# iwa-shi/CRDR

Measured on AMD Instinct MI355X. Metric: stage-3 training img/s at 256x256, higher is better.
Workload: dtype fp32; 1 GPU; config/crdr_stage_3.yaml -b 16: full GAN step (G + 5x CLIC21GVAE D + LPIPS-Alex, random-init weights), rate index cycled 0..4; global_batch=16, crop=256, parallelism=dp1

## Files before the change

crdr_amd/csrc/igemm.hip:

```cpp
#include <algorithm>
#include <type_traits>

#include "algo_id.hpp"
#include "igemm_kernel.hpp"
#include "wino.hpp"

namespace crdr {

extern template __global__ void igemm_kernel<4, 1, 1, 1, false, 0, false>(const IgemmArgs, const IgemmTaps, const IgemmGroup);
extern template __global__ void igemm_kernel<4, 1, 1, 2, false, 0, false>(const IgemmArgs, const IgemmTaps, const IgemmGroup);
extern template __global__ void igemm_kernel<4, 1, 1, 3, false, 0, false>(const IgemmArgs, const IgemmTaps, const IgemmGroup);
extern template __global__ void igemm_kernel<4, 1, 1, 4, false, 0, false>(const IgemmArgs, const IgemmTaps, const IgemmGroup);
extern template __global__ void igemm_kernel<4, 1, 1, 5, false, 0, false>(const IgemmArgs, const IgemmTaps, const IgemmGroup);
extern template __global__ void igemm_kernel<4, 1, 1, 6, false, 0, false>(const IgemmArgs, const IgemmTaps, const IgemmGroup);
extern template __global__ void igemm_kernel<4, 1, 1, 7, false, 0, false>(const IgemmArgs, const IgemmTaps, const IgemmGroup);
extern template __global__ void igemm_kernel<4, 1, 2, 2, false, 0, false>(const IgemmArgs, const IgemmTaps, const IgemmGroup);
extern template __global__ void igemm_kernel<4, 1, 2, 3, false, 0, false>(const IgemmArgs, const IgemmTaps, const IgemmGroup);
extern template __global__ void igemm_kernel<4, 1, 2, 4, false, 0, false>(const IgemmArgs, const IgemmTaps, const IgemmGroup);
extern template __global__ void igemm_kernel<2, 2, 2, 2, false, 0, false>(const IgemmArgs, const IgemmTaps, const IgemmGroup);
extern template __global__ void igemm_kernel<2, 2, 1, 1, false, 0, false>(const IgemmArgs, const IgemmTaps, const IgemmGroup);
extern template __global__ void igemm_kernel<2, 2, 1, 2, false, 0, false>(const IgemmArgs, const IgemmTaps, const IgemmGroup);
extern template __global__ void igemm_kernel<2, 2, 1, 3, false, 0, false>(const IgemmArgs, const IgemmTaps, const IgemmGroup);
extern template __global__ void igemm_kernel<2, 2, 1, 4, false, 0, false>(const IgemmArgs, const IgemmTaps, const IgemmGroup);
extern template __global__ void igemm_kernel<1, 4, 1, 1, false, 0, false>(const IgemmArgs, const IgemmTaps, const IgemmGroup);
extern template __global__ void igemm_kernel<1, 4, 1, 2, false, 0, false>(const IgemmArgs, const IgemmTaps, const IgemmGroup);
extern template __global__ void igemm_kernel<4, 2, 1, 1, false, 0, false>(const IgemmArgs, const IgemmTaps, const IgemmGroup);
extern template __global__ void igemm_kernel<4, 2, 1, 2, false, 0, false>(const IgemmArgs, const IgemmTaps, const IgemmGroup);
extern template __global__ void igemm_kernel<4, 2, 1, 3, false, 0, false>(const IgemmArgs, const IgemmTaps, const IgemmGroup);
extern template __global__ void igemm_kernel<4, 2, 2, 1, false, 0, false>(const IgemmArgs, const IgemmTaps, const IgemmGroup);
extern template __global__ void igemm_kernel<4, 2, 2, 2, false, 0, false>(const IgemmArgs, const IgemmTaps, const IgemmGroup);
extern template __global__ void igemm_kernel<2, 4, 1, 1, false, 0, false>(const IgemmArgs, const IgemmTaps, const IgemmGroup);
extern template __global__ void igemm_kernel<2, 4, 2, 1, false, 0, false>(const IgemmArgs, const IgemmTaps, const IgemmGroup);
extern template __global__ void igemm_kernel<2, 4, 1, 2, false, 0, false>(const IgemmArgs, const IgemmTaps, const IgemmGroup);
extern template __global__ void igemm_kernel<2, 2, 2, 1, false, 0, false>(const IgemmArgs, const IgemmTaps, const IgemmGroup);
extern template __global__ void igemm_kernel<2, 2, 2, 3, false, 0, false>(const IgemmArgs, const IgemmTaps, const IgemmGroup);
extern template __global__ void igemm_kernel<4, 1, 1, 1, true, 0, false>(const IgemmArgs, const IgemmTaps, const IgemmGroup);
extern template __global__ void igemm_kernel<4, 1, 1, 2, true, 0, false>(const IgemmArgs, const IgemmTaps, const IgemmGroup);
extern template __global__ void igemm_kernel<4, 1, 2, 2, true, 0, false>(const IgemmArgs, const IgemmTaps, const IgemmGroup);
extern template __global__ void igemm_kernel<2, 2, 2, 2, true, 0, false>(const IgemmArgs, const IgemmTaps, const IgemmGroup);
extern template __global__ void igemm_kernel<4, 2, 1, 1, true, 0, false>(const IgemmArgs, const IgemmTaps, const IgemmGroup);
extern template __global__ void igemm_kernel<4, 2, 1, 2, true, 0, false>(const IgemmArgs, const IgemmTaps, const IgemmGroup);
extern template __global__ void igemm_kernel<4, 2, 2, 1, true, 0, false>(const IgemmArgs, const IgemmTaps, const IgemmGroup);
extern template __global__ void igemm_kernel<4, 2, 2, 2, true, 0, false>(const IgemmArgs, const IgemmTaps, const IgemmGroup);
extern template __global__ void igemm_kernel<2, 4, 2, 1, true, 0, false>(const IgemmArgs, const IgemmTaps, const IgemmGroup);
extern template __global__ void igemm_kernel<4, 1, 1, 1, false, 3, false>(const IgemmArgs, const IgemmTaps, const IgemmGroup);
extern template __global__ void igemm_kernel<4, 1, 1, 2, false, 3, false>(const IgemmArgs, const IgemmTaps, const IgemmGroup);
extern template __global__ void igemm_kernel<4, 1, 1, 3, false, 3, false>(const IgemmArgs, const IgemmTaps, const IgemmGroup);
extern template __global__ void igemm_kernel<4, 1, 1, 4, false, 3, false>(const IgemmArgs, const IgemmTaps, const IgemmGroup);
extern template __global__ void igemm_kernel<4, 1, 1, 5, false, 3, false>(const IgemmArgs, const IgemmTaps, const IgemmGroup);
extern template __global__ void igemm_kernel<4, 1, 1, 6, false, 3, false>(const IgemmArgs, const IgemmTaps, const IgemmGroup);
extern template __global__ void igemm_kernel<4, 1, 1, 7, false, 3, false>(const IgemmArgs, const IgemmTaps, const IgemmGroup);
extern template __global__ void igemm_kernel<4, 1, 2, 2, false, 3, false>(const IgemmArgs, const IgemmTaps, const IgemmGroup);
extern template __global__ void igemm_kernel<4, 1, 2, 3, false, 3, false>(const IgemmArgs, const IgemmTaps, const IgemmGroup);
extern template __global__ void igemm_kernel<4, 1, 2, 4, false, 3, false>(const IgemmArgs, const IgemmTaps, const IgemmGroup);
extern template __global__ void igemm_kernel<2, 2, 2, 2, false, 3, false>(const IgemmArgs, const IgemmTaps, const IgemmGroup);
extern template __global__ void igemm_kernel<2, 2, 1, 1, false, 3, false>(const IgemmArgs, const IgemmTaps, const IgemmGroup);
extern template __global__ void igemm_kernel<2, 2, 1, 2, false, 3, false>(const IgemmArgs, const IgemmTaps, const IgemmGroup);
extern template __global__ void igemm_kernel<2, 2, 1, 3, false, 3, false>(const IgemmArgs, const IgemmTaps, const IgemmGroup);
extern template __global__ void igemm_kernel<2, 2, 1, 4, false, 3, false>(const IgemmArgs, const IgemmTaps, const IgemmGroup);
extern template __global__ void igemm_kernel<1, 4, 1, 1, false, 3, false>(const IgemmArgs, const IgemmTaps, const IgemmGroup);
extern template __global__ void igemm_kernel<1, 4, 1, 2, false, 3, false>(const IgemmArgs, const IgemmTaps, const IgemmGroup);
extern template __global__ void igemm_kernel<4, 2, 1, 1, false, 3, false>(const IgemmArgs, const IgemmTaps, const IgemmGroup);
extern template __global__ void igemm_kernel<4, 2, 1, 2, false, 3, false>(const IgemmArgs, const IgemmTaps, const IgemmGroup);
extern template __global__ void igemm_kernel<4, 2, 1, 3, false, 3, false>(const IgemmArgs, const IgemmTaps, const IgemmGroup);
extern template __global__ void igemm_kernel<4, 2, 2, 1, false, 3, false>(const IgemmArgs, const IgemmTaps, const IgemmGroup);
extern template __global__ void igemm_kernel<4, 2, 2, 2, false, 3, false>(const IgemmArgs, const IgemmTaps, const IgemmGroup);
extern template __global__ void igemm_kernel<2, 4, 1, 1, false, 3, false>(const IgemmArgs, const IgemmTaps, const IgemmGroup);
extern template __global__ void igemm_kernel<2, 4, 2, 1, false, 3, false>(const IgemmArgs, const IgemmTaps, const IgemmGroup);
extern template __global__ void igemm_kernel<2, 4, 1, 2, false, 3, false>(const IgemmArgs, const IgemmTaps, const IgemmGroup);
extern template __global__ void igemm_kernel<2, 2, 2, 1, false, 3, false>(const IgemmArgs, const IgemmTaps, const IgemmGroup);
extern template __global__ void igemm_kernel<2, 2, 2, 3, false, 3, false>(const IgemmArgs, const IgemmTaps, const IgemmGroup);
extern template __global__ void igemm_kernel<4, 1, 1, 2, false, 6, false>(const IgemmArgs, const IgemmTaps, const IgemmGroup);
extern template __global__ void igemm_kernel<4, 1, 1, 4, false, 6, false>(const IgemmArgs, const IgemmTaps, const IgemmGroup);
extern template __global__ void igemm_kernel<2, 2, 2, 2, false, 6, false>(const IgemmArgs, const IgemmTaps, const IgemmGroup);
extern template __global__ void igemm_kernel<2, 2, 1, 1, false, 6, false>(const IgemmArgs, const IgemmTaps, const IgemmGroup);
extern template __global__ void igemm_kernel<2, 2, 1, 2, false, 6, false>(const IgemmArgs, const IgemmTaps, const IgemmGroup);
extern template __global__ void igemm_kernel<2, 2, 1, 3, false, 6, false>(const IgemmArgs, const IgemmTaps, const IgemmGroup);
extern template __global__ void igemm_kernel<4, 2, 1, 2, false, 6, false>(const IgemmArgs, const IgemmTaps, const IgemmGroup);
extern template __global__ void igemm_kernel<2, 4, 2, 1, false, 6, false>(const IgemmArgs, const IgemmTaps, const IgemmGroup);
extern template __global__ void igemm_kernel<2, 2, 2, 1, false, 6, false>(const IgemmArgs, const IgemmTaps, const IgemmGroup);
extern template __global__ void igemm_kernel<4, 1, 1, 1, false, 0, true>(const IgemmArgs, const IgemmTaps, const IgemmGroup);
extern template __global__ void igemm_kernel<4, 1, 1, 2, false, 0, true>(const IgemmArgs, const IgemmTaps, const IgemmGroup);
extern template __global__ void igemm_kernel<4, 1, 1, 3, false, 0, true>(const IgemmArgs, const IgemmTaps, const IgemmGroup);
extern template __global__ void igemm_kernel<4, 1, 1, 4, false, 0, true>(const IgemmArgs, const IgemmTaps, const IgemmGroup);
extern template __global__ void igemm_kernel<4, 1, 1, 5, false, 0, true>(const IgemmArgs, const IgemmTaps, const IgemmGroup);
extern template __global__ void igemm_kernel<4, 1, 1, 6, false, 0, true>(const IgemmArgs, const IgemmTaps, const IgemmGroup);
extern template __global__ void igemm_kernel<4, 1, 1, 7, false, 0, true>(const IgemmArgs, const IgemmTaps, const IgemmGroup);
// ... 372 lines not shown
    CRDR_REQUIRE(al16(q.x) && al16(q.w), "conv2d: x and w must be 16-byte aligned (problem %d)", g);
    CRDR_REQUIRE(!(flags & CRDR_EPI_BIAS) || q.bias, "conv2d: BIAS flag without bias (problem %d)", g);
    CRDR_REQUIRE(!(flags & CRDR_EPI_PREADD) || q.pre, "conv2d: PREADD flag without pre (problem %d)", g);
    CRDR_REQUIRE(!(flags & (CRDR_EPI_RELUMASK | CRDR_EPI_LRELUMASK)) || q.mask, "conv2d: mask flag without mask (problem %d)", g);
    CRDR_REQUIRE(!(flags & CRDR_EPI_RES) || q.res, "conv2d: RES flag without res (problem %d)", g);
    CRDR_REQUIRE(!(flags & CRDR_EPI_COLSUM) || q.cs, "conv2d: COLSUM flag without cs (problem %d)", g);
  }
  return 0;
}

static bool rows_aligned(const crdr_conv_desc* d, const crdr_conv_io* ios, int G) {
  const bool res = d->flags & CRDR_EPI_RES, gate = d->flags & CRDR_EPI_GATE, pre = d->flags & CRDR_EPI_PREADD;
  const bool mask = d->flags & (CRDR_EPI_RELUMASK | CRDR_EPI_LRELUMASK);
  bool v = d->ldy % 4 == 0 && (!res || d->ldres % 4 == 0) && (!pre || d->ldpre % 4 == 0) && (!mask || d->ldmask % 4 == 0) &&
           (!gate || (d->ldg % 4 == 0 && al16(ios[0].gx) && al16(ios[0].gt) && al16(ios[0].sig)));
  for (int g = 0; g < G; ++g) {
    const crdr_conv_io& q = ios[g];
    v = v && al16(q.y) && (!res || al16(q.res)) && (!pre || al16(q.pre)) && (!mask || al16(q.mask));
  }
  return v;
}

static bool fast_epilogue_ok(const IgemmArgs& a, bool vec_epi) {
  const long long span_px = (256 / std::max(a.GW, 1) + 2) * (long long)std::max(a.so, 1) * a.OW + a.OW;
  const long long span = span_px * std::max(std::max(a.ldy, a.ldres), a.ldmask) * 4;
  return vec_epi && a.Cout % 4 == 0 && span < (1ll << 31) && !(a.flags & (CRDR_EPI_GATE | CRDR_EPI_PREADD | CRDR_EPI_ACCUM));
}

static void bind_io(Plan* pl, const crdr_conv_io* ios, int G, void* ws, IgemmGroup* grp) {
  IgemmArgs& a = pl->a;
  const crdr_conv_io& io = ios[0];
  a.x = io.x; a.w = io.w; a.y = io.y;
  a.counters = (int*)ws;
  a.ws = (float*)ws + CRDR_CONV_TICKETS;
  a.bias = io.bias; a.vec2 = io.vec2; a.res = io.res; a.scale = io.scale; a.shift = io.shift;
  a.gx = io.gx; a.gt = io.gt; a.sig = io.sig; a.pre = io.pre; a.mask = io.mask; a.cs = io.cs;
  memset(grp, 0, sizeof(*grp));
  for (int g = 0; g < G; ++g) {
    const crdr_conv_io& q = ios[g];
    grp->x[g] = q.x; grp->w[g] = q.w; grp->y[g] = q.y; grp->bias[g] = q.bias; grp->pre[g] = q.pre; grp->mask[g] = q.mask;
    grp->res[g] = q.res; grp->cs[g] = q.cs;
  }
}

static int launch_conv(const crdr_conv_desc* d, const crdr_conv_io* ios, int G, void* ws, size_t ws_bytes, crdr_stream_t s,
                       float* ucache = nullptr, size_t ucache_bytes = 0, int ucache_valid = 0) {
  Plan pl;
  if (int rc = build_plan(d, &pl, G)) return rc;
  if (pl.a.M == 0) return 0;
  if (int rc = check_io(d, ios, G, pl.ws_bytes, ws_bytes)) return rc;
  const bool vec_epi = rows_aligned(d, ios, G);
  if (pl.stream >= 0 && !vec_epi && d->reserved == 0) {
    if (int rc = build_plan(d, &pl, G, true)) return rc;
  }
  IgemmGroup grp;
  bind_io(&pl, ios, G, ws, &grp);
  IgemmArgs& a = pl.a;
  a.vec_epi = vec_epi ? 1 : 0;
  a.fast_epi = fast_epilogue_ok(a, vec_epi) ? 1 : 0;
  if (pl.wino != WinoKernel::None) {
    const bool f4 = pl.wino == WinoKernel::F4;
    void* prof = profile_begin(as_stream(s));
    if (f4) {
      const size_t u_bytes = wino4_workspace(d, G, 1);
      float* u = (float*)ws + CRDR_CONV_TICKETS;
      if (ucache) {
        CRDR_REQUIRE(ucache_bytes >= u_bytes, "conv2d: filter cache of %zu bytes, the launch needs %zu", ucache_bytes, u_bytes);
        u = ucache;
      }
      float* slabs = (float*)ws + CRDR_CONV_TICKETS + u_bytes / 4;
      if (int rc = wino4_launch(d, a, pl.t, grp, G, u, slabs, a.nsplit, ucache && ucache_valid, as_stream(s))) return rc;
    } else if (int rc = wino_launch(d, pl.wino == WinoKernel::F2Pairs, a, pl.t, grp, G, (float*)ws + CRDR_CONV_TICKETS, as_stream(s))) return rc;
    profile_end(f4 ? (d->kh == 5 ? 6 : 5) : 3, G * crdr_conv2d_flops(d), prof, as_stream(s));
    return 0;
  }
  if (pl.stream >= 0) {
    CRDR_REQUIRE(a.vec_epi, "conv2d: the streaming kernel needs 16-byte aligned operand rows");
    void* prof = profile_begin(as_stream(s));
    stream_launch(pl.stream, a, pl.sa, grp, pl.grid.x, pl.lds, as_stream(s));
    CRDR_CHECK_LAUNCH("gemm1x1_kernel");
    profile_end(0, G * crdr_conv2d_flops(d), prof, as_stream(s));
    return 0;
  }
  const TileCfg& t = kCfgs[pl.cfg];
  const TileForm form = a.smallc ? kTapMajor : ((d->flags & CRDR_CONV_BF16X3) ? kBf3 : ((d->flags & CRDR_CONV_BF16X6) ? kBf6 : ((a.fast_epi && a.nsplit == 1) ? kFast : kPlain)));
  const IgemmKern kern = t.kern[form];
  CRDR_REQUIRE(kern, "conv2d: config %d has no kernel for this precision", pl.cfg);
  static std::atomic<bool> attr_done[kNumTileForms][64];
  allow_full_lds(attr_done[form][pl.cfg], kern);
  void* prof = profile_begin(as_stream(s));
  hipLaunchKernelGGL(kern, pl.grid, dim3(64 * t.wm * t.wn), pl.lds, as_stream(s), a, pl.t, grp);
  CRDR_CHECK_LAUNCH("igemm_kernel");
  profile_end(0, G * crdr_conv2d_flops(d), prof, as_stream(s));
  return 0;
}

extern "C" int crdr_conv2d(const crdr_conv_desc* d, const crdr_conv_io* io, void* ws, size_t ws_bytes,
                           crdr_stream_t s) {
  CRDR_REQUIRE(d && io, "conv2d: null descriptor");
  return launch_conv(d, io, 1, ws, ws_bytes, s);
}

extern "C" int crdr_conv2d_grouped(const crdr_conv_desc* d, const crdr_conv_io* ios, int G, void* ws, size_t ws_bytes,
                                   crdr_stream_t s) {
  CRDR_REQUIRE(d && ios, "conv2d_grouped: null descriptor");
  CRDR_REQUIRE(G >= 1 && G <= CRDR_MAX_GROUP, "conv2d_grouped: %d problems (1..%d)", G, CRDR_MAX_GROUP);
  return launch_conv(d, ios, G, ws, ws_bytes, s);
}

extern "C" size_t crdr_conv2d_filter_cache_bytes(const crdr_conv_desc* d, int G) {
  Plan pl;
  if (!d || G < 1 || G > CRDR_MAX_GROUP || build_plan(d, &pl, G) || pl.wino != WinoKernel::F4) return 0;
  return wino4_workspace(d, G, 1);
}

extern "C" int crdr_conv2d_filter_item(const crdr_conv_desc* d, int G, crdr_w4_filter_item* item) {
  CRDR_REQUIRE(d && item, "conv2d_filter_item: null pointer");
  CRDR_REQUIRE(G >= 1 && G <= CRDR_MAX_GROUP, "conv2d_filter_item: %d problems (1..%d)", G, CRDR_MAX_GROUP);
  Plan pl;
  if (int rc = build_plan(d, &pl, G)) return rc;
  CRDR_REQUIRE(pl.wino == WinoKernel::F4, "conv2d_filter_item: the descriptor's `reserved` does not force the F(4x4, 3x3) kernel");
  return wino4_filter_item(d, pl.t, G, item);
}

extern "C" int crdr_w4_filters_batched(const crdr_w4_filter_item* items, const int64_t* prefix, const int64_t* meta, crdr_stream_t s) {
  CRDR_REQUIRE(items && prefix && meta, "w4_filters_batched: null pointer");
  return wino4_filters_batched(items, reinterpret_cast<const long long*>(prefix), reinterpret_cast<const long long*>(meta), as_stream(s));
}

extern "C" int crdr_conv2d_grouped_ex(const crdr_conv_desc* d, const crdr_conv_io* ios, int G, void* ws, size_t ws_bytes, float* filter_cache,
                                      size_t filter_cache_bytes, int filter_cache_valid, crdr_stream_t s) {
  CRDR_REQUIRE(d && ios, "conv2d_grouped_ex: null descriptor");
  CRDR_REQUIRE(G >= 1 && G <= CRDR_MAX_GROUP, "conv2d_grouped_ex: %d problems (1..%d)", G, CRDR_MAX_GROUP);
  CRDR_REQUIRE(!filter_cache || (reinterpret_cast<uintptr_t>(filter_cache) & 15) == 0, "conv2d_grouped_ex: the filter cache must be 16-byte aligned");
  return launch_conv(d, ios, G, ws, ws_bytes, s, filter_cache, filter_cache_bytes, filter_cache_valid);
}
```

crdr_amd/hip/lib.py:

```python
from __future__ import annotations

import ctypes as C
import os
import subprocess
import threading

_HERE = os.path.dirname(os.path.abspath(__file__))
CSRC_DIR = os.path.normpath(os.path.join(_HERE, "..", "csrc"))
LIB_PATH = os.environ.get("CRDR_HIP_LIB") or os.path.normpath(os.path.join(_HERE, "..", "_lib", "libcrdr_hip.so"))

c_float_p = C.POINTER(C.c_float)
c_void_p = C.c_void_p


class ConvDesc(C.Structure):
    _fields_ = [(n, C.c_int32) for n in (
        "N", "H", "W", "C", "OH", "OW", "OC", "kh", "kw", "stride", "pad", "transposed", "ldx", "ldy",
        "wrows", "wcols", "flags", "ldres", "ldg", "wlayout", "reserved", "ldpre", "ldmask")]


class ConvIO(C.Structure):
    _fields_ = [(n, c_void_p) for n in (
        "x", "w", "y", "bias", "vec2", "res", "scale", "shift", "gx", "gt", "sig", "pre", "mask", "cs")]

# ... 12 lines not shown
class EbwdDesc(C.Structure):
    _fields_ = [("M", C.c_int64)] + [(n, C.c_int32) for n in (
        "C", "flags", "lddout", "ldout", "lddz", "ldgres", "ldg")]


class WgradJob(C.Structure):
    _fields_ = [("slab", c_void_p), ("g", c_void_p)] + [(n, C.c_int32) for n in (
        "PC", "QC", "gI", "gJ", "T", "nsplit", "smallj", "accumulate", "gJtot", "reserved")]


class LinearGroup(C.Structure):
    _fields_ = [(n, c_void_p * 16) for n in ("w", "b", "y", "dy", "dw", "db")] + [("O", C.c_int32 * 16)]


class PackItem(C.Structure):
    _fields_ = [("src", c_void_p), ("dst", c_void_p)] + [(n, C.c_int32) for n in (
        "I", "J", "T", "rows", "cols", "mode", "srcJ", "dld")] + [("tstride", C.c_int64)]


class W4FilterItem(C.Structure):
    _fields_ = [("w", c_void_p * 16), ("u", c_void_p)] + [(n, C.c_int32) for n in (
        "G", "Cin", "Cout", "wrows", "wcols", "kchunks", "ntile", "nvar")] + [("widx", (C.c_int32 * 9) * 4), ("units", C.c_int64)]


class GdnDesc(C.Structure):
    _fields_ = [("M", C.c_int64)] + [(n, C.c_int32) for n in ("C", "ldx", "ldy", "inverse")] + [
        ("beta_min", C.c_float), ("reparam_offset", C.c_float)]


class ChannelNormDesc(C.Structure):
    _fields_ = [("M", C.c_int64)] + [(n, C.c_int32) for n in ("C", "ldx", "ldy", "ldres", "act")] + [
        ("slope", C.c_float), ("eps", C.c_float)]


class InstanceNormDesc(C.Structure):
    _fields_ = [("HW", C.c_int64)] + [(n, C.c_int32) for n in ("N", "C", "ldx", "ldy", "act")] + [("slope", C.c_float), ("eps", C.c_float)]


class GanLossDesc(C.Structure):
    _fields_ = [("n", C.c_int64), ("nq", C.c_int64), ("kind", C.c_int32), ("center", C.c_int32), ("target", C.c_float), ("sgn", C.c_float)]


class Upsample16Desc(C.Structure):
    _fields_ = [(n, C.c_int32) for n in ("N", "h", "w", "Cc", "ldi", "ldc", "ldo", "mode")]


class GcDesc2(C.Structure):
    _fields_ = [(n, C.c_int32) for n in ("N", "HW", "C", "ldy", "ldmu", "ldsigma", "ldyhat", "ldyhat2", "ldnoise", "ldlik",
                                         "ldgrad", "lddyhat", "Ctot", "c0")] + [
        ("scale_bound", C.c_float), ("likelihood_bound", C.c_float)]


class GcIO(C.Structure):
    _fields_ = [(n, c_void_p) for n in ("y", "mu", "sigma", "noise", "philox", "yhat", "yhat2", "lik_noisy", "lik_quant",
                                        "bits_noisy", "bits_quant", "gbits", "dyhat", "dy", "dmu", "dsigma", "ws")] + [
        ("ws_bytes", C.c_size_t)]


class EbwdIO(C.Structure):
    _fields_ = [(n, c_void_p) for n in (
        "dout", "out", "vec2", "scale", "shift", "gt", "sig", "dz", "gres", "dgt", "colsums", "dbias_accum")]


class GcDesc(C.Structure):
    _fields_ = [(n, C.c_int32) for n in ("N", "HW", "C", "ldy", "ldmu", "ldsigma", "ldyhat")] + [
        ("scale_bound", C.c_float), ("likelihood_bound", C.c_float)]


EPI_BIAS, EPI_RELU, EPI_LRELU, EPI_VEC2, EPI_RES, EPI_GATE, EPI_AFFINE, EPI_ACCUM = 1, 2, 4, 8, 16, 32, 64, 128
EPI_PREADD, EPI_RELUMASK, EPI_LRELUMASK, EPI_MASKOFF, EPI_COLSUM = 256, 512, 1024, 2048, 4096
CONV_NOSPLIT, CONV_BF16X3, WGRAD_BF16X3 = 8192, 16384, 1 << 16
CONV_BF16X6, WGRAD_BF16X6 = 32768, 1 << 17
WGRAD_SQUARE_Q = 1 << 18
MAX_GROUP = 16
EB_PARAMS = 58

_I, _I64, _F, _D, _P, _SZ = C.c_int, C.c_int64, C.c_float, C.c_double, c_void_p, C.c_size_t
SIGNATURES = {
    "crdr_last_error": (C.c_char_p, []),
    "crdr_version": (_I, []),
    "crdr_arch": (C.c_char_p, []),
    "crdr_profile_enable": (None, [_I]),
    "crdr_profile_read": (_I, [_I, C.POINTER(C.c_double), C.POINTER(C.c_double), C.POINTER(C.c_longlong)]),
    "crdr_conv2d_num_configs": (_I, []),
    "crdr_conv2d_num_stream_configs": (_I, []),
    "crdr_conv2d_num_wino_configs": (_I, []),
    "crdr_conv2d_wgrad_num_configs": (_I, []),
    "crdr_conv2d_wgrad_num_wino_configs": (_I, []),
    "crdr_conv2d_workspace": (_SZ, [C.POINTER(ConvDesc)]),
    "crdr_conv2d_choose_algo": (_I, [C.POINTER(ConvDesc), _I]),
    "crdr_conv2d": (_I, [C.POINTER(ConvDesc), C.POINTER(ConvIO), _P, _SZ, _P]),
    "crdr_conv2d_flops": (_D, [C.POINTER(ConvDesc)]),
    "crdr_conv2d_colsum_layout": (_I, [C.POINTER(ConvDesc), _I, C.POINTER(C.c_int), C.POINTER(C.c_int)]),
    "crdr_colsum_slab_rows": (_I, []),
    "crdr_colsum_finish_batched": (_I, [_P, _P, _P, _P, _P, _P]),
    "crdr_conv2d_grouped_workspace": (_SZ, [C.POINTER(ConvDesc), _I]),
    "crdr_conv2d_grouped": (_I, [C.POINTER(ConvDesc), _P, _I, _P, _SZ, _P]),
    "crdr_conv2d_filter_cache_bytes": (_SZ, [C.POINTER(ConvDesc), _I]),
    "crdr_conv2d_grouped_ex": (_I, [C.POINTER(ConvDesc), _P, _I, _P, _SZ, _P, _SZ, _I, _P]),
    "crdr_conv2d_filter_item": (_I, [C.POINTER(ConvDesc), _I, C.POINTER(W4FilterItem)]),
    "crdr_w4_filters_batched": (_I, [_P, _P, _P, _P]),
    "crdr_conv2d_wgrad_grouped_workspace": (_SZ, [C.POINTER(WgradDesc), _I]),
    "crdr_conv2d_wgrad_partial_grouped": (_I, [C.POINTER(WgradDesc), _P, _P, _P, _I, _P, _SZ, _P, _P]),
    "crdr_pack_weight_item": (_I, [C.POINTER(PackItem), _P]),
    "crdr_colsum_scatter": (_I, [_P, _I, _I64, _I, _I, _P, _I, _P, _SZ, _P]),
    "crdr_gauss_cond_fwd_workspace": (_SZ, [C.POINTER(GcDesc2)]),
    "crdr_gauss_cond_fwd2": (_I, [C.POINTER(GcDesc2), C.POINTER(GcIO), _P]),
    "crdr_gauss_cond_bwd2": (_I, [C.POINTER(GcDesc2), C.POINTER(GcIO), _P]),
    "crdr_gdn_workspace": (_SZ, [C.POINTER(GdnDesc), _I]),
    "crdr_gdn_fwd": (_I, [C.POINTER(GdnDesc), _P, _P, _P, _P, _P, _SZ, _P]),
    "crdr_gdn_bwd": (_I, [C.POINTER(GdnDesc), _P, _P, _P, _P, _I, _P, _I, _P, _P, _P, _SZ, _P]),
    "crdr_gdn_res_fwd": (_I, [C.POINTER(GdnDesc), _P, _P, _P, _P, _I, _P, _P, _SZ, _P]),
    "crdr_channel_norm_workspace": (_SZ, [C.POINTER(ChannelNormDesc)]),
    "crdr_channel_norm_fwd": (_I, [C.POINTER(ChannelNormDesc), _P, _P, _P, _P, _P, _P, _P]),
    "crdr_channel_norm_bwd": (_I, [C.POINTER(ChannelNormDesc), _P, _P, _P, _P, _P, _I, _P, _I, _P, _P, _P, _SZ, _P]),
    "crdr_instance_norm_workspace": (_SZ, [C.POINTER(InstanceNormDesc)]),
    "crdr_instance_norm_fwd": (_I, [C.POINTER(InstanceNormDesc), _P, _P, _P, _P, _P, _P, _SZ, _P]),
    "crdr_instance_norm_bwd": (_I, [C.POINTER(InstanceNormDesc), _P, _P, _P, _P, _P, _I, _P, _I, _P, _P, _P, _SZ, _P]),
    "crdr_reflect_pad_fwd": (_I, [_P, _I, _I, _I, _I, _I, _I, _I, _I, _I, _P, _I, _P]),
    "crdr_reflect_pad_bwd": (_I, [_P, _I, _I, _I, _I, _I, _I, _I, _I, _I, _P, _I, _P]),
    "crdr_pixel_shuffle_fwd": (_I, [_P, _I, _I, _I, _I, _I, _P, _I, _P]),
    "crdr_pixel_shuffle_bwd": (_I, [_P, _I, _I, _I, _I, _I, _P, _I, _P]),
    "crdr_upsample16_cat_workspace": (_SZ, [C.POINTER(Upsample16Desc)]),
    "crdr_upsample16_cat_fwd": (_I, [C.POINTER(Upsample16Desc), _P, _P, _P, _P]),
    "crdr_upsample16_cat_bwd": (_I, [C.POINTER(Upsample16Desc), _P, _P, _P, _P, _SZ, _P]),
    "crdr_gauss_symbols": (_I, [_P, _I, _P, _I, _P, _I, _P, _I, _F, _I, _I, _I, _P, _P, _P]),
    "crdr_philox_fork": (_I, [_P, _P, C.c_uint64, _P]),
    "crdr_philox_uniform": (_I, [_P, _I, _I, _I, _I, _I, _P, _I, _P]),
    "crdr_conv2d_wgrad_workspace": (_SZ, [C.POINTER(WgradDesc)]),
    "crdr_conv2d_wgrad": (_I, [C.POINTER(WgradDesc), _P, _P, _P, _P, _SZ, _P]),
    "crdr_conv2d_wgrad_partial": (_I, [C.POINTER(WgradDesc), _P, _P, _P, _P, _SZ, C.POINTER(WgradJob), _P]),
    "crdr_wgrad_reduce_batched": (_I, [_P, _P, _P, _P]),
    "crdr_pack_weight": (_I, [_P, _P, _I, _I, _I, _I, _I, _I, _P]),
    "crdr_pack_weights_batched": (_I, [_P, _P, _P, _P]),
    "crdr_epilogue_bwd_workspace": (_SZ, [C.POINTER(EbwdDesc)]),
    "crdr_epilogue_bwd": (_I, [C.POINTER(EbwdDesc), C.POINTER(EbwdIO), _P, _SZ, _P]),
    "crdr_col2im_rgb": (_I, [_P, _I, _I, _I, _I, _I, _I, _I, _I, _P, _P, _I, _I, _I, _I, _P]),
    "crdr_spectral_norm_fwd": (_I, [_P, _I, _I, _P, _P, _I, C.c_float, _P, _P, _P, _SZ, _P]),
    "crdr_spectral_norm_bwd": (_I, [_P, _P, _P, _P, _P, _I, _I, _P, _P, _SZ, _P]),
    "crdr_crop_flip_normalize": (_I, [_P, _P, _I, _I, _I, _P, _I, _P]),
    "crdr_linear_fwd": (_I, [_P, _I, _I, _I, _P, _P, _P, _I, _I, _I, _P]),
    "crdr_linear_bwd": (_I, [_P, _I, _I, _I, _P, _P, _I, _P, _I, _I, _P, _I, _P, _P, _P]),
    "crdr_linear_group_fwd": (_I, [_P, _I, _I, _I, _P, _I, _P]),
    "crdr_linear_group_bwd": (_I, [_P, _I, _I, _I, _P, _I, _P, _I, _P]),
    "crdr_affine": (_I, [_P, _I, _P, _P, _P, _I, _I64, _I, _P]),
    "crdr_colsum_workspace": (_SZ, [_I64, _I]),
    "crdr_colsum": (_I, [_P, _I, _I64, _I, _P, _I, _P, _SZ, _P]),
    "crdr_interp_ca_params": (_I, [_P, _P, _I, _I, _F, _P, _P, _P]),
    "crdr_interp_ca_params_bwd": (_I, [_P, _I, _I, _F, _P, _P, _P, _P, _P]),
    "crdr_bias_relu_slots": (_I, [_P, _I, _I64, _I, _I, _P, _P, _P]),
    "crdr_lrp": (_I, [_P, _I, _P, _I, _P, _I, _I64, _I, _P]),
    "crdr_lrp_bwd": (_I, [_P, _I, _P, _I, _P, _I, _I64, _I, _P]),
    "crdr_add_affine": (_I, [_P, _I, _P, _I, _P, _P, _P, _I, _I64, _I, _P]),
    "crdr_tanh_fwd": (_I, [_P, _I, _I64, _I, _P, _I, _P]),
    "crdr_tanh_bwd": (_I, [_P, _I, _P, _I, _I64, _I, _P, _I, _P]),
    "crdr_gauss_cond_fwd": (_I, [C.POINTER(GcDesc), _P, _P, _P, _P, _P, _P, _P, _P, _P, _P]),
    "crdr_gauss_cond_bwd": (_I, [C.POINTER(GcDesc), _P, _P, _P, _P, _P, _P, _I, _P, _P, _P, _P]),
    "crdr_entropy_bottleneck_fwd": (_I, [_P, _P, _P, _P, _I, _I, _I, _F, _P, _P, _P, _P]),
    "crdr_entropy_bottleneck_bwd": (_I, [_P, _P, _P, _I, _I, _I, _F, _P, _P, _P, _P, _P]),
    "crdr_eb_quantile_loss": (_I, [_P, _P, _P, _I, _P, _P, _P]),
    "crdr_reduce_workspace": (_SZ, [_I64]),
    "crdr_sqdiff_sum": (_I, [_P, _P, _I64, _P, _P, _SZ, _P]),
    "crdr_sqdiff_bwd": (_I, [_P, _P, _I64, _P, _F, _P, _P, _P]),
    "crdr_bce_diff_sum": (_I, [_P, _P, _I64, _F, _P, _P, _SZ, _P]),
    "crdr_bce_diff_bwd": (_I, [_P, _P, _I64, _F, _P, _F, _P, _P, _P]),
    "crdr_gan_loss_workspace": (_SZ, [_I64, _I64]),
# ... 67 lines not shown
```

include/crdr_hip.h:

```cpp
#ifndef CRDR_HIP_H
#define CRDR_HIP_H

#include <stddef.h>
#include <stdint.h>

#ifdef __cplusplus
extern "C" {
#endif

typedef void* crdr_stream_t;

const char* crdr_last_error(void);
int crdr_version(void);
const char* crdr_arch(void);
void crdr_profile_enable(int on);
int crdr_profile_read(int kind, double* flops, double* ms, long long* launches);


#define CRDR_EPI_BIAS 1
#define CRDR_EPI_RELU 2
#define CRDR_EPI_LRELU 4
#define CRDR_EPI_VEC2 8
#define CRDR_EPI_RES 16
#define CRDR_EPI_GATE 32
#define CRDR_EPI_AFFINE 64
#define CRDR_EPI_ACCUM 128
#define CRDR_EPI_PREADD 256
#define CRDR_EPI_RELUMASK 512
#define CRDR_EPI_LRELUMASK 1024
#define CRDR_EPI_MASKOFF 2048
#define CRDR_EPI_COLSUM 4096
#define CRDR_CONV_BF16X3 16384
#define CRDR_CONV_BF16X6 32768
#define CRDR_CONV_NOSPLIT 8192

typedef struct crdr_conv_desc {
  int32_t N, H, W, C;
  int32_t OH, OW, OC;
  int32_t kh, kw, stride, pad;
  int32_t transposed;
  int32_t ldx, ldy;
  int32_t wrows, wcols;
  int32_t flags;
  int32_t ldres;
  int32_t ldg;
  int32_t wlayout;
  int32_t reserved;
  int32_t ldpre;
  int32_t ldmask;
} crdr_conv_desc;

#define CRDR_CONV_TICKETS 16384

typedef struct crdr_conv_io {
  const float* x;
  const float* w;
  float* y;
  const float* bias;
  const float* vec2;
  const float* res;
  const float* scale;
  const float* shift;
  const float* gx;
  const float* gt;
  float* sig;
  const float* pre;
  const float* mask;
  float* cs;
} crdr_conv_io;

int crdr_conv2d_num_configs(void);
int crdr_conv2d_choose_algo(const crdr_conv_desc* d, int G);
int crdr_conv2d_num_stream_configs(void);
int crdr_conv2d_num_wino_configs(void);
size_t crdr_conv2d_workspace(const crdr_conv_desc* d);
int crdr_conv2d(const crdr_conv_desc* d, const crdr_conv_io* io, void* ws, size_t ws_bytes, crdr_stream_t s);
int crdr_conv2d_colsum_layout(const crdr_conv_desc* d, int G, int* rows, int* ld);
typedef struct crdr_colsum_job {
  const float* cs;
  float* out_pre;
  float* out_post;
  int32_t rows, ld, C, accumulate;
  int32_t nslab, cpad;
  int64_t scratch_off;
} crdr_colsum_job;
int crdr_colsum_slab_rows(void);
int crdr_colsum_finish_batched(const crdr_colsum_job* jobs, const int64_t* prefix_a, const int64_t* prefix_b, const int64_t* meta,
                               float* scratch, crdr_stream_t s);

#define CRDR_MAX_GROUP 16
size_t crdr_conv2d_grouped_workspace(const crdr_conv_desc* d, int G);
int crdr_conv2d_grouped(const crdr_conv_desc* d, const crdr_conv_io* ios, int G, void* ws, size_t ws_bytes, crdr_stream_t s);
size_t crdr_conv2d_filter_cache_bytes(const crdr_conv_desc* d, int G);
typedef struct crdr_w4_filter_item {
  const float* w[16];
  float* u;
  int32_t G, Cin, Cout, wrows, wcols, kchunks, ntile, nvar;
  int32_t widx[4][9];
  int64_t units;
// ... 295 lines not shown
```

Baseline: 223.5 img/s.

## Add specialized MFMA kernel for small-channel RGB first-layer forward convs

Adds a dedicated forward kernel for convolutions on 4-channel (padded RGB) inputs with 3x3 stride-1 or 5x5 stride-2 filters. It keeps all filters in LDS and has each wave stream 32-row output strips using fp32 MFMA, prefetching the next strip's input. Bias, activation and affine epilogues are fused and applied through an LDS transpose. It replaces the generic tap-major implicit-GEMM path for these first layers, which is poorly suited to tiny input channel counts. The new path is on by default and can be turned off through an environment variable or an API call.

```diff
diff --git a/crdr_amd/csrc/igemm.hip b/crdr_amd/csrc/igemm.hip
--- a/crdr_amd/csrc/igemm.hip
+++ b/crdr_amd/csrc/igemm.hip
@@ -3,6 +3,7 @@
 
 #include "algo_id.hpp"
 #include "igemm_kernel.hpp"
+#include "rgbconv.hpp"
 #include "wino.hpp"
 
 namespace crdr {
@@ -541,6 +542,13 @@
     profile_end(0, G * crdr_conv2d_flops(d), prof, as_stream(s));
     return 0;
   }
+  if (rgbconv_enabled() && rgbconv_fwd_supported(d, a)) {
+    void* prof = profile_begin(as_stream(s));
+    rgbconv_fwd_launch(d, a, grp, as_stream(s));
+    CRDR_CHECK_LAUNCH("rgbconv_fwd_kernel");
+    profile_end(0, G * crdr_conv2d_flops(d), prof, as_stream(s));
+    return 0;
+  }
   const TileCfg& t = kCfgs[pl.cfg];
   const TileForm form = a.smallc ? kTapMajor : ((d->flags & CRDR_CONV_BF16X3) ? kBf3 : ((d->flags & CRDR_CONV_BF16X6) ? kBf6 : ((a.fast_epi && a.nsplit == 1) ? kFast : kPlain)));
   const IgemmKern kern = t.kern[form];
diff --git a/crdr_amd/csrc/rgbconv.hip b/crdr_amd/csrc/rgbconv.hip
--- /dev/null
+++ b/crdr_amd/csrc/rgbconv.hip
@@ -0,0 +1,197 @@
+#include <algorithm>
+
+#include "rgbconv.hpp"
+
+namespace crdr {
+
+typedef unsigned u32x4 __attribute__((ext_vector_type(4)));
+
+static std::atomic<int> g_rgbconv_on{[] { const char* e = getenv("CRDR_RGBCONV"); return (e && atoi(e) == 0) ? 0 : 1; }()};
+bool rgbconv_enabled() { return g_rgbconv_on.load(std::memory_order_relaxed) != 0; }
+
+static constexpr int kRgbWaves = 8;
+static constexpr int kRgbFlags = CRDR_EPI_BIAS | CRDR_EPI_RELU | CRDR_EPI_LRELU | CRDR_EPI_AFFINE;
+static constexpr int rgb_groups(int kh) { return (kh * kh + 1) / 2; }
+static size_t rgb_lds_bytes(int kh, int cout) {
+  const int nblk2 = round_up(cdiv(cout, 32), 2);
+  return ((size_t)nblk2 * rgb_groups(kh) * 256 + 3 * 32 * nblk2 + (size_t)kRgbWaves * 1024) * sizeof(float);
+}
+
+template <int KH, int S, int NP>
+__global__ __launch_bounds__(64 * kRgbWaves) void rgbconv_fwd_kernel(const IgemmArgs p_, const IgemmGroup grp, const int pad) {
+  constexpr int T = KH * KH, NG = rgb_groups(KH), NT = 64 * kRgbWaves;
+  extern __shared__ __attribute__((aligned(16))) float smem[];
+  const int tid = threadIdx.x, lane = tid & 63, wave = __builtin_amdgcn_readfirstlane(tid >> 6);
+  const int frow = lane & 31, fh = lane >> 5;
+
+  IgemmArgs p = p_;
+  const int wpp = (int)gridDim.x / p.ngroup;
+  const int gidx = (int)blockIdx.x / wpp, wg = (int)blockIdx.x - gidx * wpp;
+  if (p.ngroup > 1) { p.x = grp.x[gidx]; p.w = grp.w[gidx]; p.y = grp.y[gidx]; p.bias = grp.bias[gidx]; }
+  const int f = p.flags;
+  constexpr int nblk2 = 2 * NP;
+  float* sW = smem;
+  float* sV = sW + nblk2 * NG * 256;
+  float* sC = sV + 3 * 32 * nblk2 + wave * 1024;
+  const int vld = 32 * nblk2;
+
+  const __amdgpu_buffer_rsrc_t rw = __builtin_amdgcn_make_buffer_rsrc(const_cast<float*>(p.w), 0, p.w_bytes, 0x00020000);
+  const __amdgpu_buffer_rsrc_t rx = __builtin_amdgcn_make_buffer_rsrc(const_cast<float*>(p.x), 0, (unsigned)p.x_bytes, 0x00020000);
+
+  constexpr int WU = 8;
+  const int wtotal = nblk2 * NG * 64;
+  for (int i0 = tid; i0 < wtotal; i0 += NT * WU) {
+    u32x4 v[WU];
+#pragma unroll
+    for (int u = 0; u < WU; ++u) {
+      const int i = i0 + u * NT;
+      const int l = i & 63, bg = i >> 6, j = bg / NG, g = bg - j * NG;
+      const int oc = j * 32 + (l & 31), k0 = 8 * g + 4 * (l >> 5);
+      v[u] = __builtin_amdgcn_raw_buffer_load_b128(rw, (i < wtotal && oc < p.wrows) ? (unsigned)(oc * p.wcols + k0) * 4u : kOobOffset, 0, 0);
+    }
+#pragma unroll
+    for (int u = 0; u < WU; ++u)
+      if (i0 + u * NT < wtotal) *reinterpret_cast<u32x4*>(sW + (i0 + u * NT) * 4) = v[u];
+  }
+  for (int c = tid; c < vld; c += NT) {
+    const bool live = c < p.Cout;
+    sV[c] = (live && (f & CRDR_EPI_BIAS)) ? p.bias[c] : 0.f;
+    sV[vld + c] = (live && (f & CRDR_EPI_AFFINE)) ? p.scale[c] : 1.f;
+    sV[2 * vld + c] = (live && (f & CRDR_EPI_AFFINE)) ? p.shift[c] : 0.f;
+  }
+  __syncthreads();
+
+  const int nstrips = (p.M + 31) >> 5;
+  const int per = (nstrips + wpp - 1) / wpp;
+  const int s0 = wg * per, s1 = min(nstrips, s0 + per);
+  const int ohw = p.OH * p.OW;
+
+  auto request = [&](int s, f32x4 (&a)[NG]) __attribute__((always_inline)) {
+    const int m = s * 32 + frow;
+    const bool live = m < p.M;
+    const int mm = live ? m : 0;
+    const int n = mm / ohw, rem = mm - n * ohw;
+    const int oh = rem / p.OW, ow = rem - oh * p.OW;
+    const int ih0 = oh * S - pad, iw0 = ow * S - pad;
+    const int base = ((n * p.H + ih0) * p.W + iw0) * 16;
+#pragma unroll
+    for (int g = 0; g < NG; ++g) {
+      const int t0 = 2 * g, t1 = 2 * g + 1;
+      const int r = fh ? t1 / KH : t0 / KH, c = fh ? t1 % KH : t0 % KH;
+      const bool tap_ok = fh ? (t1 < T) : true;
+      const int ih = ih0 + r, iw = iw0 + c;
+      const bool ok = live & tap_ok & ((unsigned)ih < (unsigned)p.H) & ((unsigned)iw < (unsigned)p.W);
+      a[g] = __builtin_bit_cast(f32x4, __builtin_amdgcn_raw_buffer_load_b128(rx, ok ? (unsigned)(base + (r * p.W + c) * 16) : kOobOffset, 0, 0));
+    }
+  };
+
+  f32x4 an[NG] = {};
+  if (s0 + wave < s1) request(s0 + wave, an);
+#pragma unroll
+  for (int g = 0; g < NG; ++g) asm volatile("" : "+v"(an[g]));
+  for (int s = s0 + wave; s < s1; s += kRgbWaves) {
+    f32x4 a[NG];
+#pragma unroll
+    for (int g = 0; g < NG; ++g) a[g] = an[g];
+    if (s + kRgbWaves < s1) request(s + kRgbWaves, an);
+
+    const int m0 = __builtin_amdgcn_readfirstlane(s * 32);
+    const __amdgpu_buffer_rsrc_t ry = __builtin_amdgcn_make_buffer_rsrc(p.y + (size_t)m0 * p.ldy, 0, 0x7fffffff, 0x00020000);
+
+#pragma unroll
+    for (int jb = 0; jb < nblk2; jb += 2) {
+      f32x16 acc[2];
+#pragma unroll
+      for (int j = 0; j < 2; ++j)
+#pragma unroll
+        for (int r = 0; r < 16; ++r) acc[j][r] = 0.f;
+      const float* wb = sW + jb * NG * 256 + lane * 4;
+#pragma unroll
+      for (int g = 0; g < NG; ++g) {
+        f32x4 bf[2];
+#pragma unroll
+        for (int j = 0; j < 2; ++j) bf[j] = *reinterpret_cast<const f32x4*>(wb + (j * NG + g) * 256);
+#pragma unroll
+        for (int e = 0; e < 4; ++e)
+#pragma unroll
+          for (int j = 0; j < 2; ++j) acc[j] = __builtin_amdgcn_mfma_f32_32x32x2f32(a[g][e], bf[j][e], acc[j], 0, 0, 0);
+      }
+      if (jb + 2 >= nblk2) {
+        __builtin_amdgcn_sched_barrier(0);
+#pragma unroll
+        for (int g = 0; g < NG; ++g) asm volatile("" : "+v"(an[g]));
+        __builtin_amdgcn_sched_barrier(0);
+      }
+#pragma unroll
+      for (int j = 0; j < 2; ++j) {
+#pragma unroll
+        for (int r = 0; r < 16; ++r) sC[((r & 3) + 8 * (r >> 2) + 4 * fh) * 32 + frow] = acc[j][r];
+        f32x4 o[4];
+        unsigned yoff[4];
+        int cc[4];
+#pragma unroll
+        for (int kq = 0; kq < 4; ++kq) {
+          const int q = lane + 64 * kq;
+          const int row = q >> 3, c4 = q & 7;
+          cc[kq] = (jb + j) * 32 + c4 * 4;
+          const bool ok = (m0 + row < p.M) && (cc[kq] < p.Cout);
+          yoff[kq] = ok ? (unsigned)(row * p.ldy + cc[kq]) * 4u : kOobOffset;
+          o[kq] = *reinterpret_cast<const f32x4*>(sC + row * 32 + c4 * 4);
+        }
+        if (f & CRDR_EPI_BIAS) {
+#pragma unroll
+          for (int kq = 0; kq < 4; ++kq) o[kq] += *reinterpret_cast<const f32x4*>(sV + cc[kq]);
+        }
+        if (f & CRDR_EPI_RELU) {
+#pragma unroll
+          for (int kq = 0; kq < 4; ++kq)
+#pragma unroll
+            for (int e = 0; e < 4; ++e) o[kq][e] = fmaxf(o[kq][e], 0.0f);
+        }
+        if (f & CRDR_EPI_LRELU) {
+#pragma unroll
+          for (int kq = 0; kq < 4; ++kq)
+#pragma unroll
+            for (int e = 0; e < 4; ++e) o[kq][e] = o[kq][e] > 0.0f ? o[kq][e] : 0.2f * o[kq][e];
+        }
+        if (f & CRDR_EPI_AFFINE) {
+#pragma unroll
+          for (int kq = 0; kq < 4; ++kq) {
+            const f32x4 scale4 = *reinterpret_cast<const f32x4*>(sV + vld + cc[kq]);
+            const f32x4 shift4 = *reinterpret_cast<const f32x4*>(sV + 2 * vld + cc[kq]);
+#pragma unroll
+            for (int e = 0; e < 4; ++e) o[kq][e] = o[kq][e] * scale4[e] + shift4[e];
+          }
+        }
+#pragma unroll
+        for (int kq = 0; kq < 4; ++kq) __builtin_amdgcn_raw_buffer_store_b128(__builtin_bit_cast(u32x4, o[kq]), ry, yoff[kq], 0, 0);
+      }
+    }
+  }
+}
+
+bool rgbconv_fwd_supported(const crdr_conv_desc* d, const IgemmArgs& a) {
+  const bool shape = (d->kh == 3 && d->kw == 3 && d->stride == 1) || (d->kh == 5 && d->kw == 5 && d->stride == 2);
+  return a.smallc && !d->transposed && shape && d->C == 4 && d->ldx == 4 && a.nsplit == 1 && (d->flags & ~kRgbFlags) == 0 && a.fast_epi &&
+         d->OC >= 1 && d->OC <= 256 && d->pad >= 0 && d->pad < d->kh && a.x_bytes < (1ull << 31) && (long long)32 * d->ldy * 4 < (1ll << 31);
+}
+
+void rgbconv_fwd_launch(const crdr_conv_desc* d, const IgemmArgs& a, const IgemmGroup& grp, hipStream_t s) {
+  using Kern = void (*)(const IgemmArgs, const IgemmGroup, const int);
+  static const Kern kerns[2][4] = {
+      {rgbconv_fwd_kernel<3, 1, 1>, rgbconv_fwd_kernel<3, 1, 2>, rgbconv_fwd_kernel<3, 1, 3>, rgbconv_fwd_kernel<3, 1, 4>},
+      {rgbconv_fwd_kernel<5, 2, 1>, rgbconv_fwd_kernel<5, 2, 2>, rgbconv_fwd_kernel<5, 2, 3>, rgbconv_fwd_kernel<5, 2, 4>}};
+  const int ki = d->kh == 3 ? 0 : 1, np = cdiv(d->OC, 64);
+  const Kern kern = kerns[ki][np - 1];
+  static std::atomic<bool> attr_done[2][4];
+  allow_full_lds(attr_done[ki][np - 1], kern);
+  const size_t lds = rgb_lds_bytes(d->kh, d->OC);
+  const int resident = cu_count() * (2 * lds <= 160 * 1024 ? 2 : 1);
+  const int nstrips = cdiv(a.M, 32);
+  const int wpp = std::max(1, std::min(resident / a.ngroup, cdiv(nstrips, 2 * kRgbWaves)));
+  hipLaunchKernelGGL(kern, dim3(wpp * a.ngroup), dim3(64 * kRgbWaves), lds, s, a, grp, (int)d->pad);
+}
+
+}
+
+extern "C" void crdr_rgbconv_enable(int on) { crdr::g_rgbconv_on.store(on != 0 ? 1 : 0, std::memory_order_relaxed); }
diff --git a/crdr_amd/csrc/rgbconv.hpp b/crdr_amd/csrc/rgbconv.hpp
--- /dev/null
+++ b/crdr_amd/csrc/rgbconv.hpp
@@ -0,0 +1,11 @@
+#pragma once
+
+#include "igemm_args.hpp"
+
+namespace crdr {
+
+bool rgbconv_enabled();
+bool rgbconv_fwd_supported(const crdr_conv_desc* d, const IgemmArgs& a);
+void rgbconv_fwd_launch(const crdr_conv_desc* d, const IgemmArgs& a, const IgemmGroup& grp, hipStream_t s);
+
+}
diff --git a/crdr_amd/hip/lib.py b/crdr_amd/hip/lib.py
--- a/crdr_amd/hip/lib.py
+++ b/crdr_amd/hip/lib.py
@@ -118,6 +118,7 @@
     "crdr_arch": (C.c_char_p, []),
     "crdr_profile_enable": (None, [_I]),
     "crdr_profile_read": (_I, [_I, C.POINTER(C.c_double), C.POINTER(C.c_double), C.POINTER(C.c_longlong)]),
+    "crdr_rgbconv_enable": (None, [_I]),
     "crdr_conv2d_num_configs": (_I, []),
     "crdr_conv2d_num_stream_configs": (_I, []),
     "crdr_conv2d_num_wino_configs": (_I, []),
diff --git a/include/crdr_hip.h b/include/crdr_hip.h
--- a/include/crdr_hip.h
+++ b/include/crdr_hip.h
@@ -15,6 +15,7 @@
 const char* crdr_arch(void);
 void crdr_profile_enable(int on);
 int crdr_profile_read(int kind, double* flops, double* ms, long long* launches);
+void crdr_rgbconv_enable(int on);
 
 
 #define CRDR_EPI_BIAS 1
```

Result: no change. 224.8 img/s (median of 2 runs) (+0.6%).
